# Kang-ChangWoo/audio-depth-estimation

Measured on AMD Instinct MI355X. Metric: depth-maps/sec (train step), higher is better.
Workload: dtype bf16; 1 GPU; unetbaseline_model unet_256 (ngf 64) train step, BatVisionV2-shaped 256x256, batch 32/GPU, Combined L1+SIlog loss, clip 1.0, AdamW; global_batch=32, image_size=256, launch=hipGraph, parallelism=dp1

## Files before the change

### audio-depth-estimation_amd/csrc/igemm.hip

```cpp
#include <stdarg.h>
#include <stdio.h>
#include <stdlib.h>
#include <string.h>

#include <mutex>

#include "epilogue.h"

namespace {

struct Tune {
  int bm = 0, bn = 0, ns = 0, noa = 0, nob = 0, skip = 0, patch = 1, tall = 1, pair = 1, tinycap = 4, bn_t2 = 0, onepx = 1, ring = 1, ring_sched = 1, ring_epi = 0, ring_geom = -1, ring_hs = 0, ring64n = 1, reduce_vec = 1;
};
const Tune& tune() {
  static Tune t;
  static std::once_flag once;
  std::call_once(once, [] {
    if (const char* e = getenv("ADN_IGEMM_BM")) t.bm = atoi(e);
    if (const char* e = getenv("ADN_IGEMM_BN")) t.bn = atoi(e);
    if (const char* e = getenv("ADN_IGEMM_NS")) t.ns = atoi(e);
#ifdef ADN_TIMING_KNOBS
    if (const char* e = getenv("ADN_IGEMM_NOA")) t.noa = atoi(e);
    if (const char* e = getenv("ADN_IGEMM_NOB")) t.nob = atoi(e);
    if (const char* e = getenv("ADN_IGEMM_SKIP")) t.skip = atoi(e);
#endif
    if (const char* e = getenv("ADN_IGEMM_PATCH")) t.patch = atoi(e);
    if (const char* e = getenv("ADN_IGEMM_TALL")) t.tall = atoi(e);
    if (const char* e = getenv("ADN_IGEMM_PAIR")) t.pair = atoi(e);
    if (const char* e = getenv("ADN_IGEMM_TINYCAP")) t.tinycap = atoi(e);
    if (const char* e = getenv("ADN_IGEMM_ONEPX")) t.onepx = atoi(e);
    if (const char* e = getenv("ADN_IGEMM_BN_T2")) t.bn_t2 = atoi(e);
    if (const char* e = getenv("ADN_IGEMM_RING")) t.ring = atoi(e);
    if (const char* e = getenv("ADN_IGEMM_RING_SCHED")) t.ring_sched = atoi(e);
    if (const char* e = getenv("ADN_IGEMM_RING_EPI")) t.ring_epi = atoi(e);
    if (const char* e = getenv("ADN_IGEMM_RING_GEOM")) t.ring_geom = atoi(e);
    if (const char* e = getenv("ADN_IGEMM_RING_HS")) t.ring_hs = atoi(e);
    if (const char* e = getenv("ADN_IGEMM_RING_N64")) t.ring64n = atoi(e);
    if (const char* e = getenv("ADN_IGEMM_REDUCE")) t.reduce_vec = strcmp(e, "scalar") != 0;
  });
  return t;
}

struct KParams {
  const void* in0;
  const void* in1;
  const void* w;
  int Hs, Ws, C0, C1, N;
  int ks;
  int wstride;
  int Msmall;
  int ksteps;
  int nsplit;
  int tiles_m, tiles_n;
  int epi;
  AdnEpiSeg seg[2];
  float* slab;
  unsigned rec_a, rec_b;
  int skip;
  int onepx;
  int lgW, lgH;
};


__device__ __forceinline__ int xcd_remap(int bid, int nwg) {
  const int q = nwg >> 3, r = nwg & 7, xcd = bid & 7;
  return (xcd < r ? xcd * (q + 1) : r * (q + 1) + (xcd - r) * q) + (bid >> 3);
}

template <int N>
__device__ __forceinline__ void wait_vmcnt() {
  asm volatile("s_waitcnt vmcnt(%0) lgkmcnt(0)" ::"n"(N) : "memory");
}

template <int BM, int BN, int NWN, int NTHR>
struct TileEpi {
  static constexpr int NW = NTHR / 64;
  static constexpr int WN = BN / NWN;
  static constexpr int NT = WN / 16, MT = 4;
  static constexpr int CPR = BN / 8;
  static constexpr int RSTEP = NTHR / CPR;
  static constexpr int RPT = BM / RSTEP;
  static constexpr int LDC = BN + 4;
  static constexpr int lds_bytes = BM * LDC * 4;
};
enum class EpiPre { None, All, NoOld };
template <int RPT, EpiPre PRE>
struct EpiPreRegs {
  u32x4_t r[PRE == EpiPre::None ? 1 : RPT], o[PRE == EpiPre::All ? RPT : 1], z[PRE == EpiPre::None ? 1 : RPT];
};

template <int BM, int BN, int NWN, int NTHR, EpiPre PRE, typename RowOp>
__device__ __forceinline__ void tile_epi_prefetch(const KParams& p, int tile_n, RowOp row_op,
                                                  EpiPreRegs<TileEpi<BM, BN, NWN, NTHR>::RPT, PRE>& pre) {
  using E = TileEpi<BM, BN, NWN, NTHR>;
  if constexpr (PRE != EpiPre::None) {
    const int tid = threadIdx.x;
    const int n0 = tile_n * BN + (tid % E::CPR) * 8, rsub = tid / E::CPR;
    const bool first = n0 < p.seg[0].channels;
    const AdnEpiSeg& sq = first ? p.seg[0] : p.seg[1];
    const int nl0 = first ? n0 : n0 - p.seg[0].channels;
#pragma unroll
    for (int k = 0; k < E::RPT; ++k) {
      pre.r[k] = pre.z[k] = u32x4_t{0u, 0u, 0u, 0u};
      if constexpr (PRE == EpiPre::All) pre.o[k] = u32x4_t{0u, 0u, 0u, 0u};
      int64_t op;
      if (row_op(rsub + E::RSTEP * k, op)) {
        const int64_t idx = op * sq.channels + nl0;
        pre.r[k] = *reinterpret_cast<const u32x4_t*>(reinterpret_cast<const uint16_t*>(sq.ref) + idx);
        if constexpr (PRE == EpiPre::All) {
          if (sq.accumulate) pre.o[k] = *reinterpret_cast<const u32x4_t*>(reinterpret_cast<const uint16_t*>(sq.out0) + idx);
        }
        if (sq.partials) pre.z[k] = *reinterpret_cast<const u32x4_t*>(reinterpret_cast<const uint16_t*>(sq.z) + idx);
      }
    }
  }
}

template <typename T, int BM, int BN, int NWN, int NTHR, EpiPre PRE, typename RowOp>
__device__ __forceinline__ void tile_epi_finish(char* smem, const KParams& p, const f32x4_t (&acc)[4][BN / NWN / 16], int tile_n,
                                                int64_t prow, RowOp row_op, float* slab, bool pre_on,
                                                const EpiPreRegs<TileEpi<BM, BN, NWN, NTHR>::RPT, PRE>& pre) {
  using E = TileEpi<BM, BN, NWN, NTHR>;
  const int tid = threadIdx.x, lane = tid & 63;
  const int wave = __builtin_amdgcn_readfirstlane(tid >> 6);
  const int wm = wave / NWN, wn = wave % NWN;
  const int frow = lane & 15, fq = lane >> 4;
  __syncthreads();
  float* ct = reinterpret_cast<float*>(smem);
#pragma unroll
  for (int i = 0; i < E::MT; ++i)
#pragma unroll
    for (int j = 0; j < E::NT; ++j)
#pragma unroll
      for (int r = 0; r < 4; ++r)
        ct[(wm * 64 + i * 16 + 4 * fq + r) * E::LDC + wn * E::WN + j * 16 + frow] = acc[i][j][r];
  __syncthreads();

  const int cg = tid % E::CPR, rsub = tid / E::CPR;
  const int n0 = tile_n * BN + cg * 8;
  int epi = p.epi;
  AdnEpiSeg sg;
  int nl;
  if (slab != nullptr) {
    epi = ADN_EPI_RAW;
    sg = p.seg[0];
    sg.out0 = slab;
    sg.channels = p.N;
    sg.partials = nullptr;
    nl = n0;
  } else if (n0 < p.seg[0].channels) {
    sg = p.seg[0];
    nl = n0;
  } else {
    sg = p.seg[1];
    nl = n0 - p.seg[0].channels;
  }
  EpiCols cols;
  epi_cols_init<T>(epi, sg, nl, cols);
  float s1[8], s2[8];
#pragma unroll
  for (int e = 0; e < 8; ++e) s1[e] = s2[e] = 0.f;

#pragma unroll
  for (int k = 0; k < E::RPT; ++k) {
    const int row = rsub + E::RSTEP * k;
    int64_t op;
    if (!row_op(row, op)) continue;
    float v[8];
    const f32x4_t v0 = *reinterpret_cast<const f32x4_t*>(ct + row * E::LDC + cg * 8);
    const f32x4_t v1 = *reinterpret_cast<const f32x4_t*>(ct + row * E::LDC + cg * 8 + 4);
#pragma unroll
    for (int e = 0; e < 4; ++e) {
      v[e] = v0[e];
      v[4 + e] = v1[e];
    }
    if constexpr (PRE != EpiPre::None) {
      if (pre_on) {
        if constexpr (PRE == EpiPre::NoOld) {
          u32x4_t old = {0u, 0u, 0u, 0u};
          if (sg.accumulate) old = *reinterpret_cast<const u32x4_t*>(reinterpret_cast<const uint16_t*>(sg.out0) + op * sg.channels + nl);
          epi_bwd_pre8(sg, cols, op, nl, v, pre.r[k], old, pre.z[k], s1, s2);
        } else {
          epi_bwd_pre8(sg, cols, op, nl, v, pre.r[k], pre.o[k], pre.z[k], s1, s2);
        }
        continue;
      }
    }
    epi_vec8<T>(epi, sg, cols, op, nl, v, s1, s2);
  }

// ... 347 lines not shown
    int iy, ix;
    bool ok0, ok1;
    int img = 0;
    if constexpr (S2) {
      const int par = q / ((TH + 1) * MW), rem = q - par * ((TH + 1) * MW);
      const int hr = rem / MW;
      int m = rem - hr * MW;
      if constexpr (PAIR) {
        img = m >= 9 ? 1 : 0;
        m -= 9 * img;
      }
      iy = 2 * oy0 - 1 + 2 * hr;
      ix = 2 * ox0 - 1 + 2 * m + par;
      const bool okx = (unsigned)ix < (unsigned)Wg && q < SEG_PIX;
      ok0 = okx && (unsigned)iy < (unsigned)Hg;
      ok1 = okx && (unsigned)(iy + 1) < (unsigned)Hg;
    } else {
      const int hr = q / MW;
      int m = q - hr * MW;
      if constexpr (PAIR) {
        img = m >= 9 ? 1 : 0;
        m -= 9 * img;
      }
      iy = oy0 + hr + (S1 ? -1 : ymin);
      ix = ox0 + m + (S1 ? -1 : xmin);
      ok0 = ok1 = (unsigned)ix < (unsigned)Wg && (unsigned)iy < (unsigned)Hg && q < SEG_PIX;
    }
    ppix[k] = (unsigned)(((tb + img) * Hg + iy) * Wg + ix + bshift);
    pmask |= (ok0 ? 1u : 0u) << (2 * k) | (ok1 ? 2u : 0u) << (2 * k);
  }
  unsigned bvo[BK_];
  const int ktot = p.wstride;
#pragma unroll
  for (int k = 0; k < BK_; ++k) {
    const int pid = wave + 4 * k;
    const int tsel = pid / BPT, row = (pid % BPT) * 16 + (lane >> 2);
    const int lc = (lane & 3) ^ (((row >> 2) & 1) << 1);
    bvo[k] = (unsigned)(((tile_n * BN + row) * ktot + tsel * Cin + lc * 8) * 2);
  }
  typedef __attribute__((address_space(3))) void* lptr_t;
  const __amdgpu_buffer_rsrc_t rs0 = __builtin_amdgcn_make_buffer_rsrc(
      (void*)(reinterpret_cast<const char*>(p.in0) - (int64_t)bshift * p.C0 * 2), 0, p.rec_a, 0x00020000);
  const __amdgpu_buffer_rsrc_t rs1 = __builtin_amdgcn_make_buffer_rsrc(
      (void*)(reinterpret_cast<const char*>(p.C1 ? p.in1 : p.in0) - (int64_t)bshift * p.C1 * 2), 0, p.rec_a, 0x00020000);
  const __amdgpu_buffer_rsrc_t rsw = __builtin_amdgcn_make_buffer_rsrc(
      (void*)(reinterpret_cast<const char*>(p.w) + ((S2 || S1) ? 0 : (int64_t)phase * p.N * ktot * 2)), 0, p.rec_b,
      0x00020000);

  const int nchunks = Cin >> 5;
  const int nseg = S2 ? 2 * nchunks : nchunks;
  const int nsteps = nseg * SEG_STEPS;

  auto issue_patch = [&](int sg, int ss) {
    const int c = S2 ? sg >> 1 : sg, par = S2 ? sg & 1 : 0;
    const int c0 = c << 5;
    const bool second = c0 >= p.C0;
    const int Cs = second ? p.C1 : p.C0;
    const int coff = second ? c0 - p.C0 : c0;
    const int soff = (par * Wg * Cs + coff) * 2;
    char* dst = Pl + (sg & 1) * PBUF + wave * 1024;
#pragma unroll
    for (int k = 0; k < PK; ++k) {
      if (k % SEG_STEPS != ss) continue;
      if (wave + 4 * k >= PPIECES) continue;
      const bool ok = (pmask >> (2 * k + par)) & 1u;
      const unsigned lc16 = (unsigned)(((lane & 3) ^ (((lane >> 4) & 1) << 1)) << 4);
      const unsigned vo = ok ? ppix[k] * (unsigned)(Cs * 2) + lc16 : OOB;
      if (second) __builtin_amdgcn_raw_ptr_buffer_load_lds(rs1, (lptr_t)(dst + k * 4096), 16, vo, soff, 0, 0);
      else __builtin_amdgcn_raw_ptr_buffer_load_lds(rs0, (lptr_t)(dst + k * 4096), 16, vo, soff, 0, 0);
    }
  };
  auto issue_b = [&](int s) {
    const int sg = s / SEG_STEPS, ss = s - sg * SEG_STEPS;
    int c, t0;
    if constexpr (S2) {
      c = sg >> 1;
      const int ky = 2 * (ss >> 1) + (sg & 1);
      t0 = ky * 4 + 2 * (ss & 1);
    } else {
      c = sg;
      t0 = TPS * ss;
    }
    const int soff = (t0 * Cin + (c << 5)) * 2;
    char* dst = Bl + (s & 1) * BBUF + wave * 1024;
#pragma unroll
    for (int k = 0; k < BK_; ++k) __builtin_amdgcn_raw_ptr_buffer_load_lds(rsw, (lptr_t)(dst + k * 4096), 16, bvo[k], soff, 0, 0);
  };

  f32x4_t acc[MT][NT];
#pragma unroll
  for (int i = 0; i < MT; ++i)
#pragma unroll
    for (int j = 0; j < NT; ++j) acc[i][j] = f32x4_t{0.f, 0.f, 0.f, 0.f};

  auto row_op = [&](int row, int64_t& op) -> bool {
    const int oy = oy0 + (row >> 4);
    const int ox = PAIR ? (row & 7) : ox0 + (row & 15);
    const int ib = PAIR ? tb + ((row >> 3) & 1) : tb;
    if constexpr (S2 || S1) op = ((int64_t)ib * Hs + oy) * Ws + ox;
    else op = ((int64_t)ib * Hl + 2 * oy + ph) * Wl + 2 * ox + pw;
    return true;
  };
  constexpr EpiPre EPRE = !PRE ? EpiPre::None : ((S2 || S1) ? EpiPre::NoOld : EpiPre::All);
  const bool pre_on = PRE && p.epi == ADN_EPI_BWD;
  EpiPreRegs<Cfg::Epi::RPT, EPRE> pre;
  if (pre_on) tile_epi_prefetch<BM, BN, NWN, NTHR, EPRE>(p, tile_n, row_op, pre);

#pragma unroll
  for (int ss = 0; ss < SEG_STEPS; ++ss) issue_patch(0, ss);
  issue_b(0);

  const int frow = lane & 15, fq = lane >> 4;
  const int qb0 = wm * 4 * MW + frow + (PAIR ? (frow >> 3) : 0);

  int s = 0;
  for (int sg = 0; sg < nseg; ++sg) {
    const char* Pb = Pl + (sg & 1) * PBUF;
#pragma unroll
    for (int ss = 0; ss < SEG_STEPS; ++ss, ++s) {
      wait_vmcnt<0>();
      __builtin_amdgcn_s_barrier();
      asm volatile("" ::: "memory");
      if (s + 1 < nsteps) issue_b(s + 1);
      if (sg + 1 < nseg) issue_patch(sg + 1, ss);
      const char* Bb = Bl + (s & 1) * BBUF;
#pragma unroll
      for (int e = 0; e < TPS; ++e) {
        int qoff;
        if constexpr (S2) qoff = ((e * (TH + 1)) + (ss >> 1)) * MW + (ss & 1);
        else if constexpr (S1) qoff = ss * MW + e;
        else qoff = (adn_t2_dy(ph, ss) - ymin) * MW + (adn_t2_dy(pw, e) - xmin);
        u32x4_t af[MT], bf[NT];
#pragma unroll
        for (int i = 0; i < MT; ++i) {
          const int q = qb0 + i * MW + qoff;
          af[i] = *reinterpret_cast<const u32x4_t*>(Pb + q * 64 + ((fq ^ (((q >> 2) & 1) << 1)) << 4));
        }
#pragma unroll
        for (int j = 0; j < NT; ++j) {
          const int row = wn * WN + j * 16 + frow;
          bf[j] = *reinterpret_cast<const u32x4_t*>(Bb + e * (BN * 64) + row * 64 + ((fq ^ (((row >> 2) & 1) << 1)) << 4));
        }
#pragma unroll
        for (int i = 0; i < MT; ++i)
#pragma unroll
          for (int j = 0; j < NT; ++j) mma_tile<T>(af[i], bf[j], acc[i][j]);
      }
    }
  }
  tile_epi_finish<T, BM, BN, NWN, NTHR, EPRE>(smem, p, acc, tile_n, (int64_t)phase * p.tiles_m + tile_m, row_op, nullptr, pre_on, pre);
#endif
}

#include "igemm_ring.h"

template <typename T, int GEOM>
__global__ __launch_bounds__(256) void igemm_direct_kernel(KParams p) {
  const int Hs = p.Hs, Ws = p.Ws, Hl = 2 * Hs, Wl = 2 * Ws;
  const int Cin = p.C0 + p.C1;
  const int64_t mout = (GEOM == ADN_GEMM_T2) ? (int64_t)p.Msmall * 4 : (int64_t)p.Msmall;
  const int64_t total = mout * p.N;
  const T* in0 = reinterpret_cast<const T*>(p.in0);
  const T* in1 = reinterpret_cast<const T*>(p.in1);
  const T* w = reinterpret_cast<const T*>(p.w);
  for (int64_t e = (int64_t)blockIdx.x * 256 + threadIdx.x; e < total; e += (int64_t)gridDim.x * 256) {
    const int64_t op = e / p.N;
    const int n = (int)(e - op * p.N);
    float acc = 0.f;
    auto dot = [&](int64_t pix, const T* wr) {
      for (int c = 0; c < p.C0; ++c) acc += ElemTraits<T>::load(in0 + pix * p.C0 + c) * ElemTraits<T>::load(wr + c);
      for (int c = 0; c < p.C1; ++c) acc += ElemTraits<T>::load(in1 + pix * p.C1 + c) * ElemTraits<T>::load(wr + p.C0 + c);
    };
    if constexpr (GEOM == ADN_GEMM_S2) {
      const int b = (int)(op / (Hs * Ws));
      const int rem = (int)(op - (int64_t)b * (Hs * Ws));
      const int oy = rem / Ws, ox = rem - oy * Ws;
      for (int tap = 0; tap < 16; ++tap) {
        const int iy = 2 * oy - 1 + (tap >> 2), ix = 2 * ox - 1 + (tap & 3);
        if ((unsigned)iy >= (unsigned)Hl || (unsigned)ix >= (unsigned)Wl) continue;
        const int64_t pix = ((int64_t)b * Hl + iy) * Wl + ix;
        const T* wr = w + (int64_t)n * p.wstride + tap * Cin;
        dot(pix, wr);
      }
    } else if constexpr (GEOM == ADN_GEMM_S1) {
      const int b = (int)(op / (Hs * Ws));
      const int rem = (int)(op - (int64_t)b * (Hs * Ws));
      const int oy = rem / Ws, ox = rem - oy * Ws;
      const int ks = p.ks, kpad = p.ks >> 1;
      for (int tap = 0; tap < ks * ks; ++tap) {
        const int iy = oy + tap / ks - kpad, ix = ox + tap % ks - kpad;
        if ((unsigned)iy >= (unsigned)Hs || (unsigned)ix >= (unsigned)Ws) continue;
        const int64_t pix = ((int64_t)b * Hs + iy) * Ws + ix;
        const T* wr = w + (int64_t)n * p.wstride + tap * Cin;
        dot(pix, wr);
      }
    } else {
      const int b = (int)(op / ((int64_t)Hl * Wl));
      const int rem = (int)(op - (int64_t)b * Hl * Wl);
      const int oy = rem / Wl, ox = rem - oy * Wl;
      const int ph = oy & 1, pw = ox & 1, i = oy >> 1, jx = ox >> 1;
      const int phase = ph * 2 + pw;
      for (int t = 0; t < 4; ++t) {
        const int iy = i + adn_t2_dy(ph, t >> 1), ix = jx + adn_t2_dy(pw, t & 1);
        if ((unsigned)iy >= (unsigned)Hs || (unsigned)ix >= (unsigned)Ws) continue;
        const int64_t pix = ((int64_t)b * Hs + iy) * Ws + ix;
        const T* wr = w + ((int64_t)phase * p.N + n) * p.wstride + t * Cin;
        dot(pix, wr);
      }
    }
    p.slab[e] = acc;
  }
}

template <typename T>
__global__ __launch_bounds__(256) void igemm_reduce_kernel(KParams p, int64_t mout, int rb) {
  const int64_t row0 = (int64_t)blockIdx.x * rb;
  const int64_t slab_stride = mout * p.N;
  const int n = blockIdx.y * 256 + threadIdx.x;
  if (n >= p.N) return;
  const bool in0 = n < p.seg[0].channels;
  const AdnEpiSeg& sg = in0 ? p.seg[0] : p.seg[1];
  const int nl = in0 ? n : n - p.seg[0].channels;
  float s1 = 0.f, s2 = 0.f;
  for (int r = 0; r < rb; ++r) {
    const int64_t op = row0 + r;
    if (op >= mout) break;
    const float* src = p.slab + op * p.N + n;
    float v = 0.f;
#pragma unroll 8
    for (int s = 0; s < p.nsplit; ++s) v += src[s * slab_stride];
    epi_scalar<T>(p.epi, sg, op, nl, v, s1, s2);
  }
  if (sg.partials && (p.epi == ADN_EPI_Z_STATS || p.epi == ADN_EPI_BWD)) {
    sg.partials[((int64_t)blockIdx.x * 2 + 0) * sg.channels + nl] = s1;
    sg.partials[((int64_t)blockIdx.x * 2 + 1) * sg.channels + nl] = s2;
  }
}

template <int G>
__device__ __forceinline__ void slab_group_add(const float* src, int64_t slab_stride, float* v) {
  f32x4_t x[G][2];
#pragma unroll
  for (int j = 0; j < G; ++j) {
    const f32x4_t* q = reinterpret_cast<const f32x4_t*>(src + j * slab_stride);
    x[j][0] = q[0];
    x[j][1] = q[1];
  }
#pragma unroll
  for (int j = 0; j < G; ++j) {
#pragma unroll
    for (int e = 0; e < 8; ++e) v[e] += x[j][e >> 2][e & 3];
  }
}

template <typename T, int EPI>
__global__ __launch_bounds__(256) void igemm_reduce_vec_kernel(KParams p, int64_t mout, int rb) {
  constexpr bool STATS = EPI == ADN_EPI_Z_STATS || EPI == ADN_EPI_BWD;
  constexpr int GMAX = (EPI == ADN_EPI_BWD && sizeof(T) == 4) ? 2
                       : (EPI == ADN_EPI_ACT || EPI == ADN_EPI_BWD || EPI == ADN_EPI_ADD) ? 4 : 8;
  extern __shared__ float reduce_terms[];
  const int64_t row0 = (int64_t)blockIdx.x * rb;
  const int64_t slab_stride = mout * p.N;
  const int cg = threadIdx.x & 31, rstep = blockDim.x >> 5;
  const int n = blockIdx.y * 256 + cg * 8;
  if (n < p.N) {
    const bool in0 = n < p.seg[0].channels;
    const AdnEpiSeg& sg = in0 ? p.seg[0] : p.seg[1];
    const int nl = in0 ? n : n - p.seg[0].channels;
    EpiVecs8 k;
    epi_scalar8_vecs<EPI>(sg, nl, k);
    for (int r = threadIdx.x >> 5; r < rb; r += rstep) {
      const int64_t op = row0 + r;
      if (op >= mout) break;
      EpiOps8<T> ops;
      epi_scalar8_request<T, EPI>(sg, op, nl, ops);
      const float* src = p.slab + op * p.N + n;
      float v[8];
#pragma unroll
      for (int e = 0; e < 8; ++e) v[e] = 0.f;
      int s = 0;
      if constexpr (GMAX == 8) {
        for (; s + 8 <= p.nsplit; s += 8) slab_group_add<8>(src + s * slab_stride, slab_stride, v);
      }
      if constexpr (GMAX >= 4) {
        for (; s + 4 <= p.nsplit; s += 4) slab_group_add<4>(src + s * slab_stride, slab_stride, v);
      }
      for (; s + 2 <= p.nsplit; s += 2) slab_group_add<2>(src + s * slab_stride, slab_stride, v);
      if (s < p.nsplit) slab_group_add<1>(src + s * slab_stride, slab_stride, v);
      float t1[8], t2[8];
      epi_scalar8<T, EPI>(sg, k, ops, op, nl, v, t1, t2);
      if constexpr (STATS) {
        if (sg.partials) {
          f32x4_t* d1 = reinterpret_cast<f32x4_t*>(reduce_terms + r * 256 + cg * 8);
          d1[0] = f32x4_t{t1[0], t1[1], t1[2], t1[3]};
          d1[1] = f32x4_t{t1[4], t1[5], t1[6], t1[7]};
          if constexpr (EPI == ADN_EPI_BWD) {
            f32x4_t* d2 = reinterpret_cast<f32x4_t*>(reduce_terms + (rb + r) * 256 + cg * 8);
            d2[0] = f32x4_t{t2[0], t2[1], t2[2], t2[3]};
            d2[1] = f32x4_t{t2[4], t2[5], t2[6], t2[7]};
          }
        }
      }
    }
  }
  if constexpr (STATS) {
    __syncthreads();
// ... 47 lines not shown
};

int plan_columns(const AdnIgemmDesc* d, bool wide, int64_t msmall) {
  const Tune& tn = tune();
  if (tn.bn) return (tn.bn == 128 && d->N % 128 == 0) ? 128 : 64;
  int bn = (d->N % 128 == 0) ? 128 : 64;
  if (d->dtype != ADN_BF16) return bn;
  if (d->geom == ADN_GEMM_T2) bn = (tn.bn_t2 == 128 && d->N % 128 == 0) ? 128 : 64;
  const int64_t t128 = adn_cdiv(msmall, 128) * (d->N / 128);
  if (d->geom == ADN_GEMM_S2 && bn == 128 && t128 >= 256 && t128 < 512) bn = 64;
  if (d->geom == ADN_GEMM_S1 && d->ks == 3 && bn == 128 && wide && d->Hs % 8 == 0 && d->Ws % 16 == 0) {
    const bool tall_ok = d->Hs % 16 == 0 && tn.tall != 0 && msmall / 256 * (d->N / 64) >= 512;
    if (tall_ok || (t128 >= 256 && t128 < 512)) bn = 64;
  }
  return bn;
}

int plan_splits(const AdnIgemmDesc* d, int64_t tiles, int ksteps, int64_t mout) {
  const Tune& tn = tune();
  int ns = 1;
  if (tiles < 256) {
    ns = (int)(512 / tiles);
    const int max_by_k = ksteps / 2 > 0 ? ksteps / 2 : 1;
    if (ns > max_by_k) ns = max_by_k;
    const bool bf16 = d->dtype == ADN_BF16;
    int cap = bf16 ? 16 : 64;
    if (bf16 && tn.tinycap > 0) {
      const int64_t by_bytes = ((int64_t)tn.tinycap << 20) / (mout * d->N * 4);
      if (by_bytes > cap) cap = by_bytes > 64 ? 64 : (int)by_bytes;
    }
    if (ns > cap) ns = cap;
    if (ns < 1) ns = 1;
  }
  if (tn.ns >= 1 && ns > tn.ns) ns = tn.ns;
  return ns;
}

void plan_unsplit(Plan* pl, Kind kind, int bm, int bn, int64_t msmall, int N) {
  pl->kind = kind;
  pl->bm = bm;
  pl->bn = bn;
  pl->tiles_m = (int)(msmall / bm);
  pl->tiles_n = N / bn;
  pl->nsplit = 1;
  pl->partial_rows = (int64_t)pl->tiles_m * pl->phases;
  pl->slab_bytes = 0;
}

void make_plan(const AdnIgemmDesc* d, Plan* pl) {
  const Tune& tn = tune();
  const bool bf16 = d->dtype == ADN_BF16;
  const int esz = bf16 ? 2 : 4;
  const int bk = 128 / esz;
  const int Cin = d->C0 + d->C1;
  const int64_t msmall = (int64_t)d->B * d->Hs * d->Ws;
  pl->phases = d->geom == ADN_GEMM_T2 ? 4 : 1;
  pl->mout = msmall * pl->phases;
  const int taps = d->geom == ADN_GEMM_S2 ? 16 : (d->geom == ADN_GEMM_T2 ? 4 : d->ks * d->ks);
  pl->wstride = d->geom == ADN_GEMM_S1 ? (int)(adn_cdiv((int64_t)taps * Cin, bk) * bk) : taps * Cin;
  const int epc = 16 / esz;
  pl->wide = (d->C0 % bk == 0) && (d->C1 % bk == 0);
  const bool narrow_ok = (d->C1 == 0) && (d->C0 % epc == 0) && (d->geom == ADN_GEMM_S1 || (taps * Cin) % bk == 0);
  const bool aligned = (pl->wide || narrow_ok) && (d->N % 64 == 0) && (d->seg[0].channels % 64 == 0) &&
                       (d->seg[1].channels % 64 == 0);
  pl->tall = pl->pair = pl->onepx = false;
  pl->rb = reduce_rows(pl->mout, d->N);
  if (!aligned) {
    pl->kind = Kind::Direct;
    pl->bm = pl->bn = 0;
    pl->nsplit = 1;
    pl->tiles_m = pl->tiles_n = 0;
    pl->ksteps = 0;
    pl->partial_rows = adn_cdiv(pl->mout, pl->rb);
    pl->slab_bytes = pl->mout * d->N * 4;
    return;
  }
  const int bn0 = (d->N % 128 == 0) ? 128 : 64;
  const bool fills256 = adn_cdiv(msmall, 256) * (d->N / bn0) * pl->phases >= 256;
  int bm = (fills256 && (bn0 == 64 || taps * Cin / bk >= 32)) ? 256 : 128;
  if (tn.bm) bm = tn.bm == 256 ? 256 : 128;
  const int bn = plan_columns(d, pl->wide, msmall);
  pl->ksteps = pl->wstride / bk;
  pl->onepx = bf16 && pl->wide && d->Hs == 1 && d->Ws == 1 && d->geom != ADN_GEMM_S1 && tn.onepx != 0;
  if (pl->onepx) pl->ksteps = (d->geom == ADN_GEMM_S2 ? 4 : 1) * (Cin / bk);
  const int64_t tile_tiles = adn_cdiv(msmall, bm) * (d->N / bn) * pl->phases;
  const int ns = plan_splits(d, tile_tiles, pl->ksteps, pl->mout);
  const bool k4 = d->geom == ADN_GEMM_S2 || d->geom == ADN_GEMM_T2;

  const bool pair = bf16 && pl->wide && d->geom == ADN_GEMM_T2 && d->Hs == 8 && d->Ws == 8 && d->B % 2 == 0 &&
                    d->N % 128 == 0 && tn.pair != 0 && tn.patch != 0 &&
                    msmall / 128 * (d->N / 128) * pl->phases >= 128;
  const bool ring = bf16 && pl->wide && ns == 1 && !pair && k4 && d->Hs % 16 == 0 && d->Ws % 16 == 0 &&
                    (d->N % 128 == 0 || (d->N == 64 && tn.ring64n != 0)) && (d->geom == ADN_GEMM_S2 || Cin % 128 == 0) &&
                    tn.ring != 0 && pl->mout * d->N < (1ll << 31) && (d->epi == ADN_EPI_Z_STATS || d->epi == ADN_EPI_BWD) &&
                    (tn.ring_epi == 0 || tn.ring_epi == d->epi) && (tn.ring_geom < 0 || tn.ring_geom == d->geom) &&
                    (tn.ring_hs == 0 || tn.ring_hs == d->Hs);
  const bool patch = bf16 && pl->wide && ns == 1 && (d->geom != ADN_GEMM_S1 || d->ks == 3) && d->Hs % 8 == 0 &&
                     d->Ws % 16 == 0 && tn.patch != 0;

  if (pair) {
    plan_unsplit(pl, Kind::Patch, 128, 128, msmall, d->N);
    pl->pair = true;
  } else if (ring) {
    const int64_t t128 = msmall / 256 * (d->N / 128) * pl->phases;
    const int rbn = (d->N == 64 || tn.ring == 64 || (tn.ring != 128 && t128 < 192)) ? 64 : 128;
    plan_unsplit(pl, Kind::Ring, 256, rbn, msmall, d->N);
  } else if (patch) {
    pl->tall = bn == 64 && d->geom != ADN_GEMM_S2 && d->Hs % 16 == 0 && tn.tall != 0 &&
               msmall / 256 * (d->N / bn) * pl->phases >= 512;
    plan_unsplit(pl, Kind::Patch, pl->tall ? 256 : 128, bn, msmall, d->N);
  } else {
    pl->kind = Kind::Tile;
    pl->bm = bm;
    pl->bn = bn;
    pl->tiles_m = (int)adn_cdiv(msmall, bm);
    pl->tiles_n = d->N / bn;
    pl->nsplit = ns;
    pl->partial_rows = ns > 1 ? adn_cdiv(pl->mout, pl->rb) : (int64_t)pl->tiles_m * pl->phases;
    pl->slab_bytes = ns > 1 ? (int64_t)ns * pl->mout * d->N * 4 : 0;
  }
}

template <typename T, int BM_, int BN, int NWN, int GEOM, bool WIDE>
void launch_mfma(const KParams& kp, const Plan& pl, hipStream_t st) {
  constexpr int lds = TileCfg<BM_, BN, NWN>::lds_bytes;
  dim3 grid(pl.tiles_m * pl.tiles_n * pl.phases, 1, pl.nsplit);
  ADN_SET_LDS_ONCE(lds, &igemm_mfma_kernel<T, BM_, BN, NWN, GEOM, WIDE>);
  hipLaunchKernelGGL((igemm_mfma_kernel<T, BM_, BN, NWN, GEOM, WIDE>), grid, dim3(BM_ * NWN), lds, st, kp);
}

template <typename T, int GEOM, bool WIDE>
void dispatch_mfma2(const KParams& kp, const Plan& pl, hipStream_t st) {
  if (pl.bm == 256) {
    if (pl.bn == 128) launch_mfma<T, 256, 128, 2, GEOM, WIDE>(kp, pl, st);
    else launch_mfma<T, 256, 64, 1, GEOM, WIDE>(kp, pl, st);
  } else {
    if (pl.bn == 128) launch_mfma<T, 128, 128, 2, GEOM, WIDE>(kp, pl, st);
    else launch_mfma<T, 128, 64, 2, GEOM, WIDE>(kp, pl, st);
  }
}
template <typename T, int GEOM>
void dispatch_mfma(const KParams& kp, const Plan& pl, hipStream_t st) {
  if (pl.wide) dispatch_mfma2<T, GEOM, true>(kp, pl, st);
  else dispatch_mfma2<T, GEOM, false>(kp, pl, st);
}

template <int BN, int GEOM, bool TALL = false, bool PRE = true, bool PAIR = false>
void launch_patch1(const KParams& kp, const Plan& pl, hipStream_t st) {
  constexpr int lds = PatchCfg<BN, GEOM, TALL, PAIR>::lds_bytes;
  ADN_SET_LDS_ONCE(lds, &igemm_patch_kernel<BN, GEOM, TALL, PRE, PAIR>);
  dim3 grid(pl.tiles_m * pl.tiles_n * pl.phases, 1, 1);
  hipLaunchKernelGGL((igemm_patch_kernel<BN, GEOM, TALL, PRE, PAIR>), grid, dim3(256), lds, st, kp);
}
inline void launch_patch(const KParams& kp, const Plan& pl, int geom, hipStream_t st) {
  if (pl.pair) {
    launch_patch1<128, ADN_GEMM_T2, false, true, true>(kp, pl, st);
  } else if (geom == ADN_GEMM_S2) {
    if (pl.bn == 128 && kp.epi == ADN_EPI_BWD) launch_patch1<128, ADN_GEMM_S2>(kp, pl, st);
    else if (pl.bn == 128) launch_patch1<128, ADN_GEMM_S2, false, false>(kp, pl, st);
    else launch_patch1<64, ADN_GEMM_S2>(kp, pl, st);
  } else if (geom == ADN_GEMM_T2) {
    if (pl.bn == 128) launch_patch1<128, ADN_GEMM_T2>(kp, pl, st);
    else if (pl.tall && kp.epi == ADN_EPI_BWD) launch_patch1<64, ADN_GEMM_T2, true, true>(kp, pl, st);
    else if (pl.tall) launch_patch1<64, ADN_GEMM_T2, true, false>(kp, pl, st);
    else launch_patch1<64, ADN_GEMM_T2>(kp, pl, st);
  } else {
    if (pl.bn == 128) launch_patch1<128, ADN_GEMM_S1>(kp, pl, st);
    else if (pl.tall && kp.epi == ADN_EPI_BWD) launch_patch1<64, ADN_GEMM_S1, true, true>(kp, pl, st);
    else if (pl.tall) launch_patch1<64, ADN_GEMM_S1, true, false>(kp, pl, st);
    else launch_patch1<64, ADN_GEMM_S1>(kp, pl, st);
  }
}

inline int device_cus() {
  static int n = 0;
  static std::once_flag once;
  std::call_once(once, [] {
    int dev = 0;
    hipDeviceProp_t pr;
    if (hipGetDevice(&dev) == hipSuccess && hipGetDeviceProperties(&pr, dev) == hipSuccess) n = pr.multiProcessorCount;
    if (n <= 0) n = 256;
  });
  return n;
}

template <int GEOM, int BN, int SCHED>
void launch_ring1(const KParams& kp, const Plan& pl, hipStream_t st) {
  constexpr int lds = RingCfg<GEOM, BN>::lds_bytes;
  ADN_SET_LDS_ONCE(lds, &igemm_ring_kernel<GEOM, BN, SCHED>);
  const int ntiles = pl.tiles_m * pl.tiles_n * pl.phases;
  const int cus = device_cus();
  const int nwgs = ntiles < cus ? ntiles : cus;
  auto magic = [](int d) -> unsigned { return (unsigned)((1ull << 32) / (unsigned)d + 1ull); };
  const int tpr = kp.Ws >> 4, tpi = (kp.Hs >> 4) * tpr;
  hipLaunchKernelGGL((igemm_ring_kernel<GEOM, BN, SCHED>), dim3(nwgs), dim3(512), lds, st, kp, ntiles, nwgs,
                     pl.tiles_n == 1 ? 0u : magic(pl.tiles_n), tpi == 1 ? 0u : magic(tpi), tpr == 1 ? 0u : magic(tpr));
}
template <int GEOM, int BN>
void launch_ring2(const KParams& kp, const Plan& pl, hipStream_t st) {
  if (tune().ring_sched) launch_ring1<GEOM, BN, 1>(kp, pl, st);
  else launch_ring1<GEOM, BN, 0>(kp, pl, st);
}
inline void launch_ring(const KParams& kp, const Plan& pl, int geom, hipStream_t st) {
  if (geom == ADN_GEMM_S2) {
    if (pl.bn == 128) launch_ring2<ADN_GEMM_S2, 128>(kp, pl, st);
    else launch_ring2<ADN_GEMM_S2, 64>(kp, pl, st);
  } else {
    if (pl.bn == 128) launch_ring2<ADN_GEMM_T2, 128>(kp, pl, st);
    else launch_ring2<ADN_GEMM_T2, 64>(kp, pl, st);
  }
}

template <typename T>
int run(const AdnIgemmDesc* d, const Plan& pl, hipStream_t st) {
  KParams kp;
  kp.in0 = d->in0;
  kp.in1 = d->in1;
  kp.w = d->w;
  kp.Hs = d->Hs;
  kp.Ws = d->Ws;
  kp.C0 = d->C0;
  kp.C1 = d->C1;
  kp.N = d->N;
  kp.ks = d->geom == ADN_GEMM_S1 ? d->ks : 0;
  kp.wstride = pl.wstride;
  kp.Msmall = d->B * d->Hs * d->Ws;
  kp.ksteps = pl.ksteps;
  kp.onepx = pl.onepx ? 1 : 0;
  kp.nsplit = pl.nsplit;
  kp.tiles_m = pl.tiles_m;
  kp.tiles_n = pl.tiles_n;
  kp.epi = d->epi;
  kp.seg[0] = d->seg[0];
  kp.seg[1] = d->seg[1];
  kp.slab = reinterpret_cast<float*>(d->workspace);
  {
    auto lg2 = [](int v) { int l = 0; while ((1 << l) < v) ++l; return (1 << l) == v ? l : -1; };
    kp.lgW = lg2(d->Ws);
    kp.lgH = lg2(d->Hs);
    if (kp.lgW < 0 || kp.lgH < 0) kp.lgW = kp.lgH = -1;
  }
  kp.rec_a = tune().noa ? 0u : 0x7ffffff0u;
  kp.rec_b = tune().nob ? 0u : 0x7ffffff0u;
  kp.skip = tune().skip;
  auto reduce = [&]() {
    const dim3 grid((unsigned)adn_cdiv(pl.mout, pl.rb), (unsigned)adn_cdiv(d->N, 256));
    const bool stats = d->epi == ADN_EPI_Z_STATS || d->epi == ADN_EPI_BWD;
    const size_t lds = stats ? (size_t)pl.rb * 256 * sizeof(float) * (d->epi == ADN_EPI_BWD ? 2 : 1) : 0;
    auto aligned16 = [](const void* q) { return (reinterpret_cast<uintptr_t>(q) & 15) == 0; };
    bool vec = tune().reduce_vec != 0 && d->N % 8 == 0 && lds <= 65536 && aligned16(kp.slab);
    for (int s = 0; s < 2; ++s) {
      const AdnEpiSeg& g = d->seg[s];
      if (g.channels == 0) continue;
      vec = vec && g.channels % 8 == 0 && aligned16(g.out0) && aligned16(g.out1) && aligned16(g.ref) && aligned16(g.z);
    }
    if (!vec) {
      hipLaunchKernelGGL((igemm_reduce_kernel<T>), grid, dim3(256), 0, st, kp, pl.mout, pl.rb);
      return;
    }
    const dim3 block(pl.rb >= 8 ? 256 : (pl.rb > 2 ? 32 * pl.rb : 64));
    switch (d->epi) {
#define ADN_REDUCE_VEC(E) \
  case E: hipLaunchKernelGGL((igemm_reduce_vec_kernel<T, E>), grid, block, lds, st, kp, pl.mout, pl.rb); break;
      ADN_REDUCE_VEC(ADN_EPI_RAW)
      ADN_REDUCE_VEC(ADN_EPI_Z_STATS)
      ADN_REDUCE_VEC(ADN_EPI_ACT)
      ADN_REDUCE_VEC(ADN_EPI_BWD)
      ADN_REDUCE_VEC(ADN_EPI_FINAL)
      ADN_REDUCE_VEC(ADN_EPI_ADD)
#undef ADN_REDUCE_VEC
    }
  };
  switch (pl.kind) {
    case Kind::Ring:
      if constexpr (sizeof(T) == 2) launch_ring(kp, pl, d->geom, st);
      ADN_CHECK_LAUNCH();
      break;
    case Kind::Patch:
      if constexpr (sizeof(T) == 2) launch_patch(kp, pl, d->geom, st);
      ADN_CHECK_LAUNCH();
      break;
    case Kind::Tile:
      if (d->geom == ADN_GEMM_S2) dispatch_mfma<T, ADN_GEMM_S2>(kp, pl, st);
      else if (d->geom == ADN_GEMM_T2) dispatch_mfma<T, ADN_GEMM_T2>(kp, pl, st);
      else dispatch_mfma<T, ADN_GEMM_S1>(kp, pl, st);
      ADN_CHECK_LAUNCH();
      if (pl.nsplit > 1) {
        reduce();
        ADN_CHECK_LAUNCH();
      }
      break;
    case Kind::Direct: {
      const int64_t total = pl.mout * d->N;
      int64_t blocks = adn_cdiv(total, 256);
      if (blocks > 65536) blocks = 65536;
      if (d->geom == ADN_GEMM_S2)
        hipLaunchKernelGGL((igemm_direct_kernel<T, ADN_GEMM_S2>), dim3((unsigned)blocks), dim3(256), 0, st, kp);
      else if (d->geom == ADN_GEMM_T2)
        hipLaunchKernelGGL((igemm_direct_kernel<T, ADN_GEMM_T2>), dim3((unsigned)blocks), dim3(256), 0, st, kp);
      else
        hipLaunchKernelGGL((igemm_direct_kernel<T, ADN_GEMM_S1>), dim3((unsigned)blocks), dim3(256), 0, st, kp);
      ADN_CHECK_LAUNCH();
      reduce();
      ADN_CHECK_LAUNCH();
      break;
    }
  }
  return ADN_OK;
}

int validate(const AdnIgemmDesc* d) {
  ADN_CHECK_ARG(d != nullptr, "adn_igemm: null descriptor");
  ADN_CHECK_ARG(d->dtype == ADN_F32 || d->dtype == ADN_BF16, "adn_igemm: bad dtype %d", d->dtype);
  ADN_CHECK_ARG(d->geom == ADN_GEMM_S2 || d->geom == ADN_GEMM_T2 || d->geom == ADN_GEMM_S1, "adn_igemm: bad geom %d",
                d->geom);
  ADN_CHECK_ARG(d->geom != ADN_GEMM_S1 || d->ks == 1 || d->ks == 3, "adn_igemm: S1 kernel side must be 1 or 3 (got %d)",
                d->ks);
  ADN_CHECK_ARG(d->B > 0 && d->Hs > 0 && d->Ws > 0, "adn_igemm: bad shape B=%d Hs=%d Ws=%d", d->B, d->Hs, d->Ws);
  ADN_CHECK_ARG(d->C0 > 0 && d->C1 >= 0 && d->N > 0, "adn_igemm: bad channels C0=%d C1=%d N=%d", d->C0, d->C1, d->N);
  ADN_CHECK_ARG(d->in0 && d->w && (d->C1 == 0 || d->in1), "adn_igemm: null operand");
  ADN_CHECK_ARG(d->epi >= ADN_EPI_RAW && d->epi <= ADN_EPI_ADD, "adn_igemm: bad epilogue %d", d->epi);
  ADN_CHECK_ARG(d->seg[0].channels + d->seg[1].channels == d->N && d->seg[0].channels > 0 && d->seg[1].channels >= 0,
                "adn_igemm: segment channels %d+%d != N=%d", d->seg[0].channels, d->seg[1].channels, d->N);
  for (int s = 0; s < 2; ++s) {
    if (d->seg[s].channels == 0) continue;
    const AdnEpiSeg& g = d->seg[s];
    if (d->epi != ADN_EPI_ACT) ADN_CHECK_ARG(g.out0, "adn_igemm: seg %d out0 is null", s);
    if (d->epi == ADN_EPI_ACT) ADN_CHECK_ARG(g.out0 || g.out1, "adn_igemm: seg %d has no output", s);
    if (d->epi == ADN_EPI_BWD) {
      ADN_CHECK_ARG(g.ref, "adn_igemm: seg %d BWD needs ref", s);
      if (g.partials) ADN_CHECK_ARG(g.z && g.mean && g.istd, "adn_igemm: seg %d BWD stats need z/mean/istd", s);
    }
  }
  const int64_t big = (int64_t)d->B * d->Hs * d->Ws * 4;
  ADN_CHECK_ARG(big * (d->C0 + d->C1) < (1ll << 40) && big < (1ll << 31), "adn_igemm: tensor too large");
  const int64_t gpix = (int64_t)d->B * d->Hs * d->Ws * (d->geom == ADN_GEMM_S2 ? 4 : 1);
// ... 47 lines not shown
```

Before: 12770 depth-maps/s.

## Add deep-pipelined pair T2 implicit-GEMM kernel for under-filled grids

Adds a new pair-mode transposed-conv implicit-GEMM kernel that keeps a multi-slot LDS ring for weights and patches and issues asynchronous buffer-to-LDS loads several steps ahead. It is used by default when the tile count does not exceed the CU count, which targets latency-bound launches where a single shallow pipeline per workgroup leaves memory latency exposed. The cost is more LDS per workgroup, a heavily templated unrolled schedule, and added correctness risk in the wait-count and slot arithmetic.

```diff
diff --git a/audio-depth-estimation_amd/csrc/igemm.hip b/audio-depth-estimation_amd/csrc/igemm.hip
--- a/audio-depth-estimation_amd/csrc/igemm.hip
+++ b/audio-depth-estimation_amd/csrc/igemm.hip
@@ -10,7 +10,7 @@
 namespace {
 
 struct Tune {
-  int bm = 0, bn = 0, ns = 0, noa = 0, nob = 0, skip = 0, patch = 1, tall = 1, pair = 1, tinycap = 4, bn_t2 = 0, onepx = 1, ring = 1, ring_sched = 1, ring_epi = 0, ring_geom = -1, ring_hs = 0, ring64n = 1, reduce_vec = 1;
+  int bm = 0, bn = 0, ns = 0, noa = 0, nob = 0, skip = 0, patch = 1, tall = 1, pair = 1, tinycap = 4, bn_t2 = 0, onepx = 1, ring = 1, ring_sched = 1, ring_epi = 0, ring_geom = -1, ring_hs = 0, ring64n = 1, reduce_vec = 1, pair_depth = 0;
 };
 const Tune& tune() {
   static Tune t;
@@ -36,6 +36,7 @@
     if (const char* e = getenv("ADN_IGEMM_RING_GEOM")) t.ring_geom = atoi(e);
     if (const char* e = getenv("ADN_IGEMM_RING_HS")) t.ring_hs = atoi(e);
     if (const char* e = getenv("ADN_IGEMM_RING_N64")) t.ring64n = atoi(e);
+    if (const char* e = getenv("ADN_IGEMM_PAIR_DEPTH")) t.pair_depth = atoi(e);
     if (const char* e = getenv("ADN_IGEMM_REDUCE")) t.reduce_vec = strcmp(e, "scalar") != 0;
   });
   return t;
@@ -689,6 +690,7 @@
 #endif
 }
 
+#include "igemm_pair_deep.h"
 #include "igemm_ring.h"
 
 template <typename T, int GEOM>
@@ -1042,9 +1044,29 @@
   dim3 grid(pl.tiles_m * pl.tiles_n * pl.phases, 1, 1);
   hipLaunchKernelGGL((igemm_patch_kernel<BN, GEOM, TALL, PRE, PAIR>), grid, dim3(256), lds, st, kp);
 }
+inline int device_cus() {
+  static int n = 0;
+  static std::once_flag once;
+  std::call_once(once, [] {
+    int dev = 0;
+    hipDeviceProp_t pr;
+    if (hipGetDevice(&dev) == hipSuccess && hipGetDeviceProperties(&pr, dev) == hipSuccess) n = pr.multiProcessorCount;
+    if (n <= 0) n = 256;
+  });
+  return n;
+}
+
+template <int WRING, int NPB>
+void launch_pair_deep(const KParams& kp, const Plan& pl, hipStream_t st) {
+  constexpr int lds = PairDeepCfg<WRING, NPB>::lds_bytes;
+  ADN_SET_LDS_ONCE(lds, &igemm_pair_deep_kernel<WRING, NPB>);
+  dim3 grid(pl.tiles_m * pl.tiles_n * pl.phases, 1, 1);
+  hipLaunchKernelGGL((igemm_pair_deep_kernel<WRING, NPB>), grid, dim3(256), lds, st, kp);
+}
 inline void launch_patch(const KParams& kp, const Plan& pl, int geom, hipStream_t st) {
   if (pl.pair) {
-    launch_patch1<128, ADN_GEMM_T2, false, true, true>(kp, pl, st);
+    if (tune().pair_depth == 1 || pl.tiles_m * pl.tiles_n * pl.phases > device_cus()) launch_patch1<128, ADN_GEMM_T2, false, true, true>(kp, pl, st);
+    else launch_pair_deep<4, 4>(kp, pl, st);
   } else if (geom == ADN_GEMM_S2) {
     if (pl.bn == 128 && kp.epi == ADN_EPI_BWD) launch_patch1<128, ADN_GEMM_S2>(kp, pl, st);
     else if (pl.bn == 128) launch_patch1<128, ADN_GEMM_S2, false, false>(kp, pl, st);
@@ -1060,18 +1082,6 @@
     else if (pl.tall) launch_patch1<64, ADN_GEMM_S1, true, false>(kp, pl, st);
     else launch_patch1<64, ADN_GEMM_S1>(kp, pl, st);
   }
-}
-
-inline int device_cus() {
-  static int n = 0;
-  static std::once_flag once;
-  std::call_once(once, [] {
-    int dev = 0;
-    hipDeviceProp_t pr;
-    if (hipGetDevice(&dev) == hipSuccess && hipGetDeviceProperties(&pr, dev) == hipSuccess) n = pr.multiProcessorCount;
-    if (n <= 0) n = 256;
-  });
-  return n;
 }
 
 template <int GEOM, int BN, int SCHED>
diff --git a/audio-depth-estimation_amd/csrc/igemm_pair_deep.h b/audio-depth-estimation_amd/csrc/igemm_pair_deep.h
--- /dev/null
+++ b/audio-depth-estimation_amd/csrc/igemm_pair_deep.h
@@ -0,0 +1,203 @@
+#pragma once
+
+#include <type_traits>
+
+constexpr unsigned PAIR_OOB = 0x80000000u;
+
+template <int WRING_, int NPB_>
+struct PairDeepCfg {
+  using PC = PatchCfg<128, ADN_GEMM_T2, false, true>;
+  static constexpr int WRING = WRING_, NPB = NPB_;
+  static constexpr int WAHEAD = WRING - 1;
+  static constexpr int PAHEAD = NPB >= 3 ? 2 : 1;
+  static constexpr int PK = (PC::PPIECES + 3) / 4;
+  static constexpr int PSLOT = 4 * PK * 1024;
+  static constexpr int BBUF = PC::BBUF;
+  static constexpr int W_OFF = NPB * PSLOT;
+  static constexpr int stage_bytes = W_OFF + WRING * BBUF;
+  static constexpr int lds_bytes = stage_bytes > PC::Epi::lds_bytes ? stage_bytes : PC::Epi::lds_bytes;
+  static constexpr int gcd(int a, int b) { return b == 0 ? a : gcd(b, a % b); }
+  static constexpr int PERIOD = WRING * (2 * NPB) / gcd(WRING, 2 * NPB);
+  static constexpr int LEAD = (WAHEAD > 2 * PAHEAD ? WAHEAD : 2 * PAHEAD) + ((WAHEAD > 2 * PAHEAD ? WAHEAD : 2 * PAHEAD) & 1);
+  static constexpr int group(int ss) { return 4 + ((ss & 1) == 0 ? 2 : 1); }
+  static constexpr int depth(int ss) { return WAHEAD < 2 * PAHEAD - 1 + (ss & 1) ? WAHEAD : 2 * PAHEAD - 1 + (ss & 1); }
+  static constexpr int in_flight(int ss) {
+    int n = 0;
+    for (int j = 1; j < depth(ss); ++j) n += group(ss + j);
+    return n;
+  }
+  static_assert(WRING >= 2 && NPB >= 2 && PC::PPIECES == 11 && PK == 3, "pair-deep kernel: layout");
+  static_assert(lds_bytes <= LDS_MAX, "pair-deep kernel: LDS budget");
+};
+
+template <int WRING, int NPB>
+__global__ __launch_bounds__(256) void igemm_pair_deep_kernel(KParams p) {
+#if defined(__HIP_DEVICE_COMPILE__)
+  typedef uint16_t T;
+  using Cfg = PairDeepCfg<WRING, NPB>;
+  using PC = typename Cfg::PC;
+  constexpr int BN = 128, BM = PC::BM, NWN = PC::NWN, NTHR = PC::NTHR, MW = PC::MW, SEG_PIX = PC::SEG_PIX;
+  constexpr int WN = BN / NWN, NT = WN / 16, MT = 4;
+  constexpr int PK = Cfg::PK, PSLOT = Cfg::PSLOT, BBUF = Cfg::BBUF, WAHEAD = Cfg::WAHEAD, PAHEAD = Cfg::PAHEAD;
+  constexpr int BPT = BN / 16, BK_ = 2 * BPT / 4;
+  extern __shared__ __attribute__((aligned(16))) char smem[];
+  char* Pl = smem;
+  char* Bl = smem + Cfg::W_OFF;
+
+  const int tid = threadIdx.x, lane = tid & 63;
+  const int wave = __builtin_amdgcn_readfirstlane(tid >> 6);
+  const int wm = wave >> 1, wn = wave & 1;
+  const int nwg = p.tiles_m * p.tiles_n * 4;
+  const int wg0 = xcd_remap(blockIdx.x, nwg);
+  const int tile_m = wg0 % p.tiles_m;
+  const int wg = wg0 / p.tiles_m;
+  const int tile_n = wg % p.tiles_n;
+  const int phase = wg / p.tiles_n;
+  const int ph = phase >> 1, pw = phase & 1;
+  const int Hs = p.Hs, Ws = p.Ws, Hl = 2 * Hs, Wl = 2 * Ws;
+  const int Cin = p.C0 + p.C1;
+  const int tb = 2 * tile_m;
+  const int ymin = ph == 0 ? -1 : 0, xmin = pw == 0 ? -1 : 0;
+
+  unsigned ppix[PK], pdead[PK];
+  const int bshift = Ws + 1;
+#pragma unroll
+  for (int k = 0; k < PK; ++k) {
+    const int q = 16 * (wave + 4 * k) + (lane >> 2);
+    const int hr = q / MW;
+    int m = q - hr * MW;
+    const int img = m >= 9 ? 1 : 0;
+    m -= 9 * img;
+    const int iy = hr + ymin, ix = m + xmin;
+    const bool ok = (unsigned)ix < (unsigned)Ws && (unsigned)iy < (unsigned)Hs && q < SEG_PIX;
+    ppix[k] = (unsigned)(((tb + img) * Hs + iy) * Ws + ix + bshift);
+    pdead[k] = ok ? 0u : PAIR_OOB;
+  }
+  const unsigned lc16 = (unsigned)(((lane & 3) ^ (((lane >> 4) & 1) << 1)) << 4);
+  unsigned bvo[BK_];
+  const int ktot = p.wstride;
+#pragma unroll
+  for (int k = 0; k < BK_; ++k) {
+    const int pid = wave + 4 * k;
+    const int tsel = pid / BPT, row = (pid % BPT) * 16 + (lane >> 2);
+    const int lc = (lane & 3) ^ (((row >> 2) & 1) << 1);
+    bvo[k] = (unsigned)(((tile_n * BN + row) * ktot + tsel * Cin + lc * 8) * 2);
+  }
+  typedef __attribute__((address_space(3))) void* lptr_t;
+  const char* gbase0 = reinterpret_cast<const char*>(p.in0) - (int64_t)bshift * p.C0 * 2;
+  const char* gbase1 = reinterpret_cast<const char*>(p.C1 ? p.in1 : p.in0) - (int64_t)bshift * p.C1 * 2;
+  const __amdgpu_buffer_rsrc_t rsw = __builtin_amdgcn_make_buffer_rsrc(
+      (void*)(reinterpret_cast<const char*>(p.w) + (int64_t)phase * p.N * ktot * 2), 0, p.rec_b, 0x00020000);
+
+  const int nseg = Cin >> 5;
+  const int nsteps = 2 * nseg;
+
+  auto issue_group = [&](auto WSLOT, auto PB, auto SS, int sw, int sgp) {
+    constexpr int wslot = decltype(WSLOT)::value, pb = decltype(PB)::value, ss = decltype(SS)::value;
+    {
+      const bool live = (unsigned)sw < (unsigned)nsteps;
+      const unsigned dead = live ? 0u : PAIR_OOB;
+      const int soff = live ? (2 * (sw & 1) * Cin + ((sw >> 1) << 5)) * 2 : 0;
+      char* dst = Bl + wslot * BBUF + wave * 1024;
+#pragma unroll
+      for (int k = 0; k < BK_; ++k)
+        __builtin_amdgcn_raw_ptr_buffer_load_lds(rsw, (lptr_t)(dst + k * 4096), 16, bvo[k] | dead, soff, 0, 0);
+    }
+    {
+      const bool live = (unsigned)sgp < (unsigned)nseg;
+      const unsigned dead = live ? 0u : PAIR_OOB;
+      const int c0 = sgp << 5;
+      const bool second = live && c0 >= p.C0;
+      const int Cs = second ? p.C1 : p.C0;
+      const int soff = live ? (second ? c0 - p.C0 : c0) * 2 : 0;
+      const __amdgpu_buffer_rsrc_t rs = __builtin_amdgcn_make_buffer_rsrc((void*)(second ? gbase1 : gbase0), 0, p.rec_a, 0x00020000);
+      char* dst = Pl + pb * PSLOT + wave * 1024;
+#pragma unroll
+      for (int k = ss; k < PK; k += 2) {
+        const unsigned vo = ((ppix[k] * (unsigned)(Cs * 2) + lc16) & 0x7fffffffu) | pdead[k] | dead;
+        __builtin_amdgcn_raw_ptr_buffer_load_lds(rs, (lptr_t)(dst + k * 4096), 16, vo, soff, 0, 0);
+      }
+    }
+  };
+
+  f32x4_t acc[MT][NT];
+#pragma unroll
+  for (int i = 0; i < MT; ++i)
+#pragma unroll
+    for (int j = 0; j < NT; ++j) acc[i][j] = f32x4_t{0.f, 0.f, 0.f, 0.f};
+
+  auto row_op = [&](int row, int64_t& op) -> bool {
+    const int oy = row >> 4, ox = row & 7, ib = tb + ((row >> 3) & 1);
+    op = ((int64_t)ib * Hl + 2 * oy + ph) * Wl + 2 * ox + pw;
+    return true;
+  };
+  constexpr EpiPre EPRE = EpiPre::All;
+  const bool pre_on = p.epi == ADN_EPI_BWD;
+  EpiPreRegs<PC::Epi::RPT, EPRE> pre;
+  if (pre_on) tile_epi_prefetch<BM, BN, NWN, NTHR, EPRE>(p, tile_n, row_op, pre);
+
+  auto lead = [&](auto self, auto V) {
+    constexpr int v = decltype(V)::value;
+    if constexpr (v < Cfg::LEAD) {
+      constexpr int s = v - Cfg::LEAD;
+      constexpr int sw = s + WAHEAD, sgp = (s + Cfg::LEAD) / 2 - Cfg::LEAD / 2 + PAHEAD;
+      issue_group(std::integral_constant<int, (sw % WRING + WRING) % WRING>{}, std::integral_constant<int, (sgp % NPB + NPB) % NPB>{},
+                  std::integral_constant<int, v & 1>{}, sw, sgp);
+      self(self, std::integral_constant<int, v + 1>{});
+    }
+  };
+  lead(lead, std::integral_constant<int, 0>{});
+
+  const int frow = lane & 15, fq = lane >> 4;
+  const int qb0 = wm * 4 * MW + frow + (frow >> 3);
+
+  auto step = [&](auto U, int s) {
+    constexpr int u = decltype(U)::value, ss = u & 1;
+    wait_vmcnt<Cfg::in_flight(ss)>();
+    __builtin_amdgcn_s_barrier();
+    asm volatile("" ::: "memory");
+    const char* Pb = Pl + ((u >> 1) % NPB) * PSLOT;
+    const char* Bb = Bl + (u % WRING) * BBUF;
+    u32x4_t af[2][MT], bf[2][NT];
+#pragma unroll
+    for (int e = 0; e < 2; ++e) {
+      constexpr int dy = ss == 0 ? 1 : 0;
+      const int qoff = dy * MW + (e == 0 ? 1 : 0);
+#pragma unroll
+      for (int i = 0; i < MT; ++i) {
+        const int q = qb0 + i * MW + qoff;
+        af[e][i] = *reinterpret_cast<const u32x4_t*>(Pb + q * 64 + ((fq ^ (((q >> 2) & 1) << 1)) << 4));
+      }
+#pragma unroll
+      for (int j = 0; j < NT; ++j) {
+        const int row = wn * WN + j * 16 + frow;
+        bf[e][j] = *reinterpret_cast<const u32x4_t*>(Bb + e * (BN * 64) + row * 64 + ((fq ^ (((row >> 2) & 1) << 1)) << 4));
+      }
+    }
+    issue_group(std::integral_constant<int, (u + WAHEAD) % WRING>{}, std::integral_constant<int, ((u >> 1) + PAHEAD) % NPB>{},
+                std::integral_constant<int, ss>{}, s + WAHEAD, (s >> 1) + PAHEAD);
+#pragma unroll
+    for (int e = 0; e < 2; ++e)
+#pragma unroll
+      for (int i = 0; i < MT; ++i)
+#pragma unroll
+        for (int j = 0; j < NT; ++j) mma_tile<T>(af[e][i], bf[e][j], acc[i][j]);
+    __builtin_amdgcn_sched_barrier(0);
+  };
+  auto period = [&](auto self, auto U, int s0) -> bool {
+    constexpr int u = decltype(U)::value;
+    if constexpr (u < Cfg::PERIOD) {
+      step(std::integral_constant<int, u>{}, s0 + u);
+      step(std::integral_constant<int, u + 1>{}, s0 + u + 1);
+      if (s0 + u + 2 >= nsteps) return false;
+      return self(self, std::integral_constant<int, u + 2>{}, s0);
+    } else {
+      return true;
+    }
+  };
+  for (int s0 = 0; period(period, std::integral_constant<int, 0>{}, s0); s0 += Cfg::PERIOD) {
+  }
+  wait_vmcnt<0>();
+  tile_epi_finish<T, BM, BN, NWN, NTHR, EPRE>(smem, p, acc, tile_n, (int64_t)phase * p.tiles_m + tile_m, row_op, nullptr, pre_on, pre);
+#endif
+}
```

Result: no change. 12810 depth-maps/s (median of 6 runs) (+0.3%).
